# Aman-4-Real/MMTG

Measured on AMD Instinct MI355X. Metric: train tokens/sec, full MMTG config (GPT-2-base-zh decoder, 5x(img+text) 2048-d WenLan embs), higher is better.
Workload: dtype bf16; 1 GPU; Full MMTG train step: S=5 experience steps, T=15+221=236 decoder positions, GPT-2 12L/768/12H V=13317, dropout 0.1 on, MyLoss stage 3 + 0.2*KL, clip 1.0, AdamW; rows_per_gpu=64, global_rows=64, seq_len=236, parallelism=single GPU, no collective

## Files before the change

### mmtg_amd/csrc/wgrad.hip

```cpp
#include "gemm_common.h"
#include <stdlib.h>

namespace {

constexpr int WG_MAXP = 8;

struct WgProb {
    const void* A; const void* B; float* C;
    long lda, ldb, ldc;
    int M, N, tiles_m, tiles_n, tile0, m_fast;
    int bytesA, bytesB;
    int planeA, planeB;
};
struct WgArgs {
    WgProb pr[WG_MAXP];
    int n, K, kper, splits, ntiles, accumulate;
    int touch;
    float* ws;
    unsigned* cnt;
};

__device__ __forceinline__ void wg_store_band(float* C, long ldc, int M, int N, int mw0, int nw0, int h, const f32x4 (&v)[4],
                                              char* lds, int lane, bool accumulate) {
    const int g = lane >> 4, l15 = lane & 15;
// ... 283 lines not shown
    const int wr = wave >> 2, wc = wave & 3;
    int t, split, m0, n0;
    const WgProb& P = a.pr[wg_locate<256>(a, t, split, m0, n0)];
    const int M = P.M, N = P.N;
    const long lda = P.lda, ldb = P.ldb;
    const int kbeg = split * a.kper;
    const int klen = max(0, min(a.K, kbeg + a.kper) - kbeg);
    const int nk = 2 * ((klen + 127) >> 7);
    const __amdgpu_buffer_rsrc_t ra = __builtin_amdgcn_make_buffer_rsrc(const_cast<void*>(P.A), 0, P.bytesA, 0x00020000);
    const __amdgpu_buffer_rsrc_t rb = __builtin_amdgcn_make_buffer_rsrc(const_cast<void*>(P.B), 0, P.bytesB, 0x00020000);
    const int sa0 = (int)(((long)kbeg * lda + m0) * 2), sb0 = (int)(((long)kbeg * ldb + n0) * 2);
    const int stepa = (int)(64 * lda * 2), stepb = (int)(64 * ldb * 2);
    const int lA00 = wave * 1024, lA01 = (wave + 8) * 1024, lA10 = 16384 + lA00, lA11 = 16384 + lA01;
    const int lB00 = TA + lA00, lB01 = TA + lA01, lB10 = TA + lA10, lB11 = TA + lA11;
    const int vA00 = g8_voff<8>(lda, m0, M, 0, wave, lane), vA01 = g8_voff<8>(lda, m0, M, 0, wave + 8, lane);
    const int vA10 = g8_voff<8>(lda, m0, M, 1, wave, lane), vA11 = g8_voff<8>(lda, m0, M, 1, wave + 8, lane);
    const int vB00 = g8_voff<4>(ldb, n0, N, 0, wave, lane), vB01 = g8_voff<4>(ldb, n0, N, 0, wave + 8, lane);
    const int vB10 = g8_voff<4>(ldb, n0, N, 1, wave, lane), vB11 = g8_voff<4>(ldb, n0, N, 1, wave + 8, lane);
    const int kl0 = wave * 4 + (lane >> 4), kl1 = kl0 + 32;
#define G8_A0(t_) g8_issue(ra, smem + ((t_) & 1) * STAGE + lA00, smem + ((t_) & 1) * STAGE + lA01, (t_) * 64 + kl0 < klen ? vA00 : OOB, (t_) * 64 + kl1 < klen ? vA01 : OOB, sa0 + (t_) * stepa)
#define G8_A1(t_) g8_issue(ra, smem + ((t_) & 1) * STAGE + lA10, smem + ((t_) & 1) * STAGE + lA11, (t_) * 64 + kl0 < klen ? vA10 : OOB, (t_) * 64 + kl1 < klen ? vA11 : OOB, sa0 + (t_) * stepa)
#define G8_B0(t_) g8_issue(rb, smem + ((t_) & 1) * STAGE + lB00, smem + ((t_) & 1) * STAGE + lB01, (t_) * 64 + kl0 < klen ? vB00 : OOB, (t_) * 64 + kl1 < klen ? vB01 : OOB, sb0 + (t_) * stepb)
#define G8_B1(t_) g8_issue(rb, smem + ((t_) & 1) * STAGE + lB10, smem + ((t_) & 1) * STAGE + lB11, (t_) * 64 + kl0 < klen ? vB10 : OOB, (t_) * 64 + kl1 < klen ? vB11 : OOB, sb0 + (t_) * stepb)
    int oa[4], ob[2];
    ks_offsets<128, 4>(wr * 64, lane, oa);
    ks_offsets<128, 2>(wc * 32, lane, ob);
    ob[0] += TA; ob[1] += TA;

    f32x4 acc[8][4];
#pragma unroll
    for (int i = 0; i < 8; ++i)
#pragma unroll
        for (int j = 0; j < 4; ++j) acc[i][j] = f32x4{0.f, 0.f, 0.f, 0.f};

    G8_B0(0); G8_A0(0); G8_B1(0); G8_A1(0);
    G8_B0(1); G8_A0(1); G8_B1(1);
    wait_vmcnt<6>();
    asm volatile("s_barrier" ::: "memory");
    if (wr == 1) asm volatile("s_barrier" ::: "memory");

    bf16x8 fa[4][2], fb0[2][2], fb1[2][2];
#define G8_RD_A(ST, AH)                                                                                    \
    _Pragma("unroll") for (int kk = 0; kk < 2; ++kk) _Pragma("unroll") for (int i = 0; i < 4; ++i)          \
        fa[i][kk] = tr_read_pair(smem + (ST) * STAGE + (AH) * 16384, oa[i] + kk * 8192, oa[i] + kk * 8192 + 1024)
#define G8_RD_B(ST, BH, F)                                                                                 \
    _Pragma("unroll") for (int kk = 0; kk < 2; ++kk) _Pragma("unroll") for (int j = 0; j < 2; ++j)          \
        F[j][kk] = tr_read_pair(smem + (ST) * STAGE + (BH) * 16384, ob[j] + kk * 8192, ob[j] + kk * 8192 + 1024)
#define G8_TILE(ST, kt)                                                                                    \
    do {                                                                                                   \
        G8_RD_B(ST, 0, fb0);                                                                               \
        __builtin_amdgcn_sched_barrier(0);                                                                 \
        G8_RD_A(ST, 0);                                                                                    \
        G8_A1((kt) + 1);                                                                                   \
         \
        asm volatile("s_waitcnt lgkmcnt(15)" ::: "memory");                                                \
        G8_SYNC_IN(); g8_mfma<0, 0>(fa, fb0, acc); G8_SYNC_OUT();                                           \
        G8_RD_B(ST, 1, fb1);                                                                               \
        G8_B0((kt) + 2);                                                                                   \
        G8_SYNC_IN(); g8_mfma<0, 1>(fa, fb1, acc); G8_SYNC_OUT();                                           \
        G8_RD_A(ST, 1);                                                                                    \
        G8_A0((kt) + 2);                                                                                   \
        G8_SYNC_IN(); g8_mfma<1, 1>(fa, fb1, acc); G8_SYNC_OUT();                                           \
        G8_B1((kt) + 2);                                                                                   \
        wait_vmcnt<6>();                                                      \
        G8_SYNC_IN(); g8_mfma<1, 0>(fa, fb0, acc); G8_SYNC_OUT();                                           \
    } while (0)
    for (int kt = 0; kt < nk; kt += 2) {
        G8_TILE(0, kt);
        G8_TILE(1, kt + 1);
    }
#undef G8_TILE
#undef G8_RD_A
#undef G8_RD_B
#undef G8_A0
#undef G8_A1
#undef G8_B0
#undef G8_B1
    wait_vmcnt<0>();
    if (wr == 0) asm volatile("s_barrier" ::: "memory");
    asm volatile("s_barrier" ::: "memory");
    wg_reduce_store<false, 8, 256 * 256>(a, P.C, P.ldc, M, N, m0 + wr * 128, n0 + wc * 64, t, split, 8, wave, lane, acc, smem + wave * 4096);
}

}

extern "C" int mmtg_wgrad_group(int config, int n, const mmtg_wgrad_problem* probs, int K, int splits, float* ws, long ws_floats,
                                unsigned* counters, long n_counters, int accumulate, void* stream) {
    const bool x3 = (config & 2) != 0;
    const bool x3c = x3 && (config & 4) != 0;
    config &= ~6;
    MMTG_REQUIRE(config == 0 || (config == 1 && !x3),
                 "wgrad_group: config 0 (128x128 tiles), 1 (256x256 eight-phase tiles), 2 (128x128 tiles, x3 operands) or 6 (x3, combined stages)");
    const int TB = config ? 256 : 128, NWV = config ? 8 : 4, KQ = config ? 128 : 64;
    MMTG_REQUIRE(n >= 1 && n <= WG_MAXP && probs, "wgrad_group: 1..%d problems", WG_MAXP);
    MMTG_REQUIRE(K > 0 && splits >= 1, "wgrad_group: K and splits must be positive");
    WgArgs a;
    memset(&a, 0, sizeof(a));
    int tiles = 0;
    double flops = 0, bytes = 0;
    for (int i = 0; i < n; ++i) {
        const mmtg_wgrad_problem& q = probs[i];
        MMTG_REQUIRE(q.A && q.B && q.C && q.M > 0 && q.N > 0, "wgrad_group: problem %d has a null operand or an empty shape", i);
        MMTG_REQUIRE(MMTG_ALIGNED16(q.A) && MMTG_ALIGNED16(q.B) && MMTG_ALIGNED16(q.C), "wgrad_group: operands must be 16-byte aligned");
        MMTG_REQUIRE(q.lda % 8 == 0 && q.ldb % 8 == 0 && q.M % 8 == 0 && q.N % 8 == 0 && q.ldc % 4 == 0 && q.lda >= q.M && q.ldb >= q.N && q.ldc >= q.N,
                     "wgrad_group: problem %d: M, N, lda, ldb multiples of 8, ldc of 4, leading dimensions >= extents", i);
        if (x3) MMTG_REQUIRE(q.planeA % 8 == 0 && q.planeB % 8 == 0 && q.planeA >= (long)(K - 1) * q.lda + q.M && q.planeB >= (long)(K - 1) * q.ldb + q.N,
                             "wgrad_group: problem %d: an operand's lo plane must lie behind its hi plane (distance %% 8 == 0)", i);
        const long bytesA = ((x3 ? q.planeA : 0) + (long)(K - 1) * q.lda + q.M) * 2, bytesB = ((x3 ? q.planeB : 0) + (long)(K - 1) * q.ldb + q.N) * 2;
        MMTG_REQUIRE(bytesA < 0x7FFFFF00L && bytesB < 0x7FFFFF00L, "wgrad_group: operands must stay below 2 GiB");
        WgProb& p = a.pr[i];
        p.A = q.A; p.B = q.B; p.C = q.C; p.lda = q.lda; p.ldb = q.ldb; p.ldc = q.ldc; p.M = q.M; p.N = q.N;
        p.tiles_m = cdiv(q.M, TB); p.tiles_n = cdiv(q.N, TB);
        p.tile0 = tiles;
        p.m_fast = p.tiles_n > p.tiles_m;
        p.bytesA = (int)bytesA; p.bytesB = (int)bytesB;
        p.planeA = x3 ? (int)(q.planeA * 2) : 0; p.planeB = x3 ? (int)(q.planeB * 2) : 0;
        tiles += p.tiles_m * p.tiles_n;
        flops += 2.0 * q.M * q.N * (double)K;
        bytes += 2.0 * ((double)q.M * K + (double)q.N * K) + 4.0 * (double)q.M * q.N;
    }
    const int kper = cdiv(cdiv(K, splits), KQ) * KQ;
    splits = cdiv(K, kper);
    MMTG_REQUIRE(splits == 1 || (ws && counters && MMTG_ALIGNED16(ws)), "wgrad_group: split products need the workspace and the counters");
    MMTG_REQUIRE(splits == 1 || (ws_floats >= (long)tiles * splits * TB * TB && n_counters >= (long)tiles * NWV),
                 "wgrad_group: workspace needs %ld floats and %ld counters", (long)tiles * splits * TB * TB, (long)tiles * NWV);
    a.n = n; a.K = K; a.kper = kper; a.splits = splits; a.ntiles = tiles; a.accumulate = accumulate;
    a.ws = ws; a.cnt = counters;
    static const int touch = getenv("MMTG_WGRAD_TOUCH") ? atoi(getenv("MMTG_WGRAD_TOUCH")) : 0;
    a.touch = touch;
    hipStream_t s = (hipStream_t)stream;
    ProfScope prof(MMTG_PROF_GEMM_BF16, s, flops, bytes);
    static bool attr_done = false;
    static const bool fence = getenv("MMTG_WGRAD_FENCE") != nullptr;
    if (config == 1) {
        const size_t shm8 = 2 * (256 + 256) * 128;
        static bool attr8_done = false;
        if (!attr8_done) {
            if (hipFuncSetAttribute((const void*)wgrad_group_p8_kernel, hipFuncAttributeMaxDynamicSharedMemorySize, (int)shm8) != hipSuccess)
                MMTG_FAIL(MMTG_ERR_HIP, "wgrad_group: cannot raise dynamic LDS to %zu bytes", shm8);
            attr8_done = true;
        }
        hipLaunchKernelGGL(wgrad_group_p8_kernel, dim3(tiles * splits), dim3(512), shm8, s, a);
        MMTG_LAUNCH_CHECK("wgrad_group");
        return MMTG_OK;
    }
    const size_t shm = (128 + 128) * 128;
    if (!attr_done) {
        if (hipFuncSetAttribute((const void*)wgrad_group_kernel<true>, hipFuncAttributeMaxDynamicSharedMemorySize, (int)shm) != hipSuccess ||
            hipFuncSetAttribute((const void*)wgrad_group_kernel<false>, hipFuncAttributeMaxDynamicSharedMemorySize, (int)shm) != hipSuccess)
            MMTG_FAIL(MMTG_ERR_HIP, "wgrad_group: cannot raise dynamic LDS to %zu bytes", shm);
        attr_done = true;
    }
    static const int ablate = getenv("MMTG_WGRAD_ABLATE") ? atoi(getenv("MMTG_WGRAD_ABLATE")) : 0;
    if (x3c) {
        const size_t shmc = 2 * shm;
        static bool x3c_done = false;
        if (!x3c_done) {
            if (hipFuncSetAttribute((const void*)wgrad_group_kernel<false, 0, true, true>, hipFuncAttributeMaxDynamicSharedMemorySize, (int)shmc) != hipSuccess)
                MMTG_FAIL(MMTG_ERR_HIP, "wgrad_group: cannot raise dynamic LDS to %zu bytes", shmc);
            x3c_done = true;
        }
        hipLaunchKernelGGL((wgrad_group_kernel<false, 0, true, true>), dim3(tiles * splits), dim3(256), shmc, s, a);
    } else if (x3) {
        static bool x3_done = false;
        if (!x3_done) {
            if (hipFuncSetAttribute((const void*)wgrad_group_kernel<false, 0, true>, hipFuncAttributeMaxDynamicSharedMemorySize, (int)shm) != hipSuccess)
                MMTG_FAIL(MMTG_ERR_HIP, "wgrad_group: cannot raise dynamic LDS to %zu bytes", shm);
            x3_done = true;
        }
        hipLaunchKernelGGL((wgrad_group_kernel<false, 0, true>), dim3(tiles * splits), dim3(256), shm, s, a);
    } else if (ablate) {
        static bool abl_done = false;
        if (!abl_done) {
            (void)hipFuncSetAttribute((const void*)wgrad_group_kernel<false, 1>, hipFuncAttributeMaxDynamicSharedMemorySize, (int)shm);
            (void)hipFuncSetAttribute((const void*)wgrad_group_kernel<false, 2>, hipFuncAttributeMaxDynamicSharedMemorySize, (int)shm);
            abl_done = true;
        }
        if (ablate == 1) hipLaunchKernelGGL((wgrad_group_kernel<false, 1>), dim3(tiles * splits), dim3(256), shm, s, a);
        else hipLaunchKernelGGL((wgrad_group_kernel<false, 2>), dim3(tiles * splits), dim3(256), shm, s, a);
    } else if (fence) hipLaunchKernelGGL(wgrad_group_kernel<true>, dim3(tiles * splits), dim3(256), shm, s, a);
    else if (touch > 0) {
        static bool t_done = false;
        if (!t_done) { (void)hipFuncSetAttribute((const void*)wgrad_group_kernel<false, 3>, hipFuncAttributeMaxDynamicSharedMemorySize, (int)shm); t_done = true; }
        hipLaunchKernelGGL((wgrad_group_kernel<false, 3>), dim3(tiles * splits), dim3(256), shm, s, a);
    } else hipLaunchKernelGGL(wgrad_group_kernel<false>, dim3(tiles * splits), dim3(256), shm, s, a);
    MMTG_LAUNCH_CHECK("wgrad_group");
    return MMTG_OK;
}
```

### mmtg_amd/engine.py

```python
from __future__ import annotations

import contextlib
import math

import numpy as np
import torch

from . import hip
from .configs import rnn_param_shapes

ALIGN = 64


class ParamLayout:

    def __init__(self, model_cfgs, gpt2_cfg):
        S = model_cfgs["seq_len"]
        E = model_cfgs["topic"]["input_dim"]
        H = model_cfgs["topic"]["hidden_dim"]
        D = gpt2_cfg["n_embd"]
        V = gpt2_cfg["vocab_size"]
        NP = gpt2_cfg["n_positions"]
        L = gpt2_cfg["n_layer"]
        self.Vpad = (V + 127) // 128 * 128
# ... 82 lines not shown
        self.heads = model_cfgs["SELF_ATT"]["attention_heads"]
        self.P = data_cfg["topic_prompt_length"]
        self.msl = data_cfg["max_sent_length"]
        self.max_seq_length = data_cfg["max_seq_length"]
        self.two_sents = 2 * (self.msl + 2)
        self.D = gpt2_cfg["n_embd"]
        self.nH = gpt2_cfg["n_head"]
        self.L = gpt2_cfg["n_layer"]
        self.V = gpt2_cfg["vocab_size"]
        self.NP = gpt2_cfg["n_positions"]
        self.eps = gpt2_cfg.get("layer_norm_epsilon", 1e-5)
        self.pdrop = (gpt2_cfg.get("embd_pdrop", 0.1), gpt2_cfg.get("attn_pdrop", 0.1), gpt2_cfg.get("resid_pdrop", 0.1))
        self.rnn = {ch: (model_cfgs[ch]["type"], int(model_cfgs[ch]["num_layers"])) for ch in ("image", "text")}
        self.rnn_pdrop = float(model_cfgs.get("dropout", 0.0))
        for ch in ("image", "text"):
            rnn_param_shapes(model_cfgs, ch)
            if model_cfgs[ch]["input_dim"] != self.E or model_cfgs[ch]["hidden_dim"] != self.H:
                raise ValueError("The hidden dim of topic, image and text must be equal (model.py:36); this engine also takes one input dim")
        if self.D % self.nH or self.D // self.nH != 64:
            raise ValueError("the attention kernels are built for head dim 64 (n_embd=%d, n_head=%d)" % (self.D, self.nH))
        if model_cfgs["MM_ATT"]["attention_dim"] != 1:
            raise ValueError("MM_ATT.attention_dim must be 1 (the reference's broadcast at model.py:200 requires it)")


def gaussian_prior(S):
    j = np.arange(S, dtype=np.float64)
    rows = []
    for i in range(S):
        v = np.exp(-0.5 * (j - i) ** 2) / math.sqrt(2 * math.pi)
        v32 = v.astype(np.float64)
        rows.append((v32 / v32.sum()).astype(np.float32))
    return np.stack(rows)


import os as _os


def _dist_rank():
    import torch.distributed as dist
    return dist.get_rank() if dist.is_available() and dist.is_initialized() else int(_os.environ.get("RANK", "0"))


_NO_OCC4 = bool(_os.environ.get("MMTG_GEMM_NO_OCC4"))
_WG_NUM = float(_os.environ.get("MMTG_WGRAD_NUM", "760"))
_WG_CAP = int(_os.environ.get("MMTG_WGRAD_CAP", "12"))
_NO_FEW_ROWS = bool(_os.environ.get("MMTG_NO_FEW_ROWS"))
_WGRAD_SLAB = not _os.environ.get("MMTG_WGRAD_ATOMIC")
_NO_GATHER = bool(_os.environ.get("MMTG_NO_GATHER"))
_PREFETCH = int(_os.environ.get("MMTG_PREFETCH", "0"))


def _wgrad_splits(M, N, K, occ4=False, slots=512, t_iter=1.1, t_fixed=6.0):
    tiles = ((M + 127) // 128) * ((N + 127) // 128)
    if occ4 and not _NO_OCC4:
        smax = max(1, K // 256)
        s = round(_WG_NUM / tiles) if tiles < 512 else round(2520.0 / tiles)
        return int(max(1, min(smax, s, _WG_CAP)))
    best, best_t = 1, None
    for s in range(1, 33):
        if s > 1 and K // s < 256:
            break
        rounds = -(-tiles * s // slots)
        t = rounds * (K / (64.0 * s) * t_iter + t_fixed) + tiles * s * 65536 / 1.3e6
        if best_t is None or t < best_t * 0.97:
            best, best_t = s, t
    return best


_LAZY_ZERO = _os.environ.get("MMTG_FULL_ZERO_GRAD") is None
_WTE_T = _os.environ.get("MMTG_NO_WTE_T") is None
_P8T = _os.environ.get("MMTG_GEMM_P8T", "0") != "0"
_WGRAD_GROUP = _os.environ.get("MMTG_WGRAD_GROUP", "1") != "0"
_WGRAD_GROUP_SPLITS = int(_os.environ.get("MMTG_WGRAD_GROUP_SPLITS", "0"))
_GELU_GRAD = _os.environ.get("MMTG_GELU_GRAD", "0") != "0"
_DEFER_SUMS = _os.environ.get("MMTG_DEFER_SUMS", "1") != "0"
_WGRAD_TAIL = int(_os.environ.get("MMTG_WGRAD_TAIL", "8"))
_TAIL_FORK_EARLY = _os.environ.get("MMTG_WGRAD_TAIL_FORK", "loop") == "loop"
_LMHEAD_GROUP = _os.environ.get("MMTG_LMHEAD_GROUP", "1") != "0"
_LMHEAD_GROUP_SPLITS = int(_os.environ.get("MMTG_LMHEAD_GROUP_SPLITS", "0"))
_WGRAD_STREAM = _os.environ.get("MMTG_WGRAD_STREAM", "0") != "0"
_ENC_STREAMS = _os.environ.get("MMTG_ENC_STREAMS", "0") != "0"
_HYBRID_ENC_BF16 = _os.environ.get("MMTG_HYBRID_ENC_BF16", "1") != "0"
_X3_WG_CFG = 6 if _os.environ.get("MMTG_WGRAD_X3_COMBINED", "1") != "0" else 2
_WGRAD_GROUP_CFG = int(_os.environ.get("MMTG_WGRAD_GROUP_CFG", "0"))


def _group_splits(tiles, K, slots=1024):
    if _WGRAD_GROUP_SPLITS > 0:
        return _WGRAD_GROUP_SPLITS
    return int(max(1, min(slots // max(1, tiles), K // 1024, 16)))


def _group_splits_x3(tiles, K):
    if _X3_WG_CFG != 6:
        return _group_splits(tiles, K)
    if _WGRAD_GROUP_SPLITS > 0:
        return _WGRAD_GROUP_SPLITS
    s = 512 // max(1, tiles)
    if s == 0:
        s = 2048 // tiles
    return int(max(1, min(s, K // 1024, 16)))


def _wgrad_splits_p8(M, N, K, cus=256):
    if not _P8T or K % 128 or M < 256 or N < 256:
        return None
    tiles = ((M + 255) // 256) * ((N + 255) // 256)
    if tiles > cus // 2:
        return None
    units = K // 128
    s0 = max(1, min(cus // tiles, units // 4))
    per = -(-units // s0)
    return -(-units // per)


def _round_capacity(n):
    if n <= 1024:
        return 1024
    k = 1 << (int(n - 1).bit_length() - 1)
    for q in (4, 5, 6, 7, 8):
        if k * q // 4 >= n:
            return k * q // 4
    return 2 * k


def mix_seed(seed, site):
    x = (seed ^ (0x9E3779B9 * (site + 1))) & 0xFFFFFFFF
    x = ((x ^ (x >> 16)) * 0x7FEB352D) & 0xFFFFFFFF
    x = ((x ^ (x >> 15)) * 0x846CA68B) & 0xFFFFFFFF
    return (x ^ (x >> 16)) & 0xFFFFFFFF


def initial_drop_seed(rank=0):
    return mix_seed(torch.initial_seed() & 0xFFFFFFFF, 0x5EED + 7919 * rank)


class Engine:

    def __init__(self, model_cfgs, data_cfg, gpt2_cfg, master, table, dtype=hip.BF16, x3=False, hybrid=False):
        hip.lib()
        if x3 and dtype != hip.F32:
            raise ValueError("the split-precision (bf16x3) products belong to fp32 storage")
        if hybrid and not x3:
            raise ValueError("the hybrid mode (bf16x3f) is the split-precision forward with a bf16 backward: it needs x3")
        if not master.is_cuda:
            raise RuntimeError("the MMTG engine runs on an MI355X (cuda) device only -- there is no CPU path")
        self.sh = Shapes(model_cfgs, data_cfg, gpt2_cfg)
        if x3 and self.sh.D % 128:
            raise ValueError("compute_dtype='bf16x3' needs n_embd to be a multiple of 128 (got %d): use compute_dtype='f32'" % self.sh.D)
        self.layout = ParamLayout(model_cfgs, gpt2_cfg)
        assert master.numel() == self.layout.total and master.dtype == torch.float32
        self.dev = master.device
        self.dtype = dtype
        self.tdt = hip.torch_dtype(dtype)
        self.master = master
        self.grad = None
        self.wc = master if dtype == hip.F32 else torch.zeros(self.layout.total, device=self.dev, dtype=torch.bfloat16)
        self.x3 = bool(x3)
        self.hybrid = bool(hybrid)
        self.wc2 = torch.zeros(2, self.layout.total, device=self.dev, dtype=torch.bfloat16) if self.x3 else None
        self.copies_fresh = dtype == hip.F32 and not self.x3
        self._init_transposed()
        self.set_table(table)
        self.prior = torch.from_numpy(gaussian_prior(self.sh.S)).to(self.dev)
        self.ws = {}
        self._ws_tag = ""
        self.act = None
# ... 703 lines not shown
            xb = self.buf("x_cond_b", tuple(a["x"].shape), torch.bfloat16)
            hip.cast_f32_to(a["x"], xb, a["x"].numel())
        ab.update(x3=False, px3=False, gelu_grad=False, elem_mask=True, layers=layers, x_last=a["x_last_b"], hf=hi(a["hf"]), h1=h1b, x=xb, ids32=None)
        try:
            with self._as_bf16():
                self.act = ab
                seg = self._backward_decoder(ab, dlogits)
        finally:
            self.act = a
        if _HYBRID_ENC_BF16:
            ae = self._encoder_record_bf16(a)
            with self._as_bf16():
                self._backward_encoder(ae, seg, dkl)
            return
        seg32 = self.buf("d_seg32", tuple(seg.shape), torch.float32)
        hip.cast_to_f32(seg, seg32, seg.numel())
        self._backward_encoder(a, seg32, dkl)

    def _encoder_record_bf16(self, a):
        def cast(t, name):
            b = self.buf("hyb_" + name, tuple(t.shape), torch.bfloat16)
            hip.cast_f32_to(t, b, t.numel())
            return b
        ae = dict(a)
        for k in ("o", "t_ln", "t_raw", "xt"):
            ae[k] = cast(a[k], k)
        ae["alpha"] = {mod: (cast(q, "aqkv_" + mod), cast(c, "actx_" + mod), p) for mod, (q, c, p) in a["alpha"].items()}
        enc = {}
        for ch, (layers, h_ln) in a["enc"].items():
            recs = []
            for l, rec in enumerate(layers):
                r = dict(rec)
                r["h"] = cast(rec["h"], "h_%s%d" % (ch, l))
                r["inp"] = recs[l - 1]["h"] if (l > 0 and rec["inp"] is layers[l - 1]["h"]) else cast(rec["inp"], "inp_%s%d" % (ch, l))
                recs.append(r)
            enc[ch] = (recs, cast(h_ln, "hln_" + ch))
        ae["enc"] = enc
        return ae

    def backward(self, dlogits, dkl=0.0):
        a = self.act
        self.ensure_grad()
        if self._lazy is not None and not self.wgrad_overwrite:
            self.grad.zero_()
            self._lazy = None
        if self.hybrid and a.get("x3"):
            self._backward_hybrid(dlogits, dkl)
        else:
            self._backward_encoder(a, self._backward_decoder(a, dlogits), dkl)
        if self._tail_side is not None:
            torch.cuda.current_stream().wait_stream(self._tail_side)
            self._tail_side = None
        self._lazy = None

    def _backward_decoder(self, a, dlogits):
        sh = self.sh
        B, T, M, L = a["B"], a["T"], a["M"], a["L"]
        S, E, H, D, P = sh.S, sh.E, sh.H, sh.D, sh.P
        pe, pa, pr = a["pdrop"]
        Vp = self.layout.Vpad
        pre = "decoder.gpt2.transformer."
        dhf = self.buf("d_hf", (M, D))
        x3 = bool(a.get("x3"))
        if x3:
            dlp = dlogits if isinstance(dlogits, hip.Planes) else hip.split_planes(dlogits, M, Vp, self.pbuf("dlogits_p", M, Vp))
            hip.gemm_x3(dlp, hip.Planes(self.wte_t, D, Vp), dhf, M, D, Vp)
            tiles = hip.wgrad_group_sizes(((Vp, D),), 1, 0)[0]
            hs = _LMHEAD_GROUP_SPLITS or _group_splits_x3(tiles, M)
            _, nws, ncnt = hip.wgrad_group_sizes(((Vp, D),), hs, 0)
            hws = self.buf("wgrad_group_ws_head", (nws,), torch.float32) if hs > 1 else None
            hcnt = self.ws.get(("wgrad_group_cnt", torch.int32))
            if hcnt is None or hcnt.numel() < ncnt:
                hcnt = self.ws[("wgrad_group_cnt", torch.int32)] = torch.zeros(ncnt, device=self.dev, dtype=torch.int32)
            hip.wgrad_group([(dlp, a["hf"], self.Gp("wte"), Vp, D, Vp, D, D)], M, hs, hws, hcnt, accumulate=not self.wgrad_overwrite, config=_X3_WG_CFG)
            if self.wgrad_overwrite and self._ow_rec is not None:
                self._ow_rec[1].append((self.layout.pack_range["wte"][0], Vp * D))
        elif getattr(self, "wte_t", None) is not None and Vp % 128 == 0 and not self.x3:
            hip.gemm(dlogits, self.wte_t, dhf, M, D, Vp, transB=True, ldb=Vp)
        else:
            hip.gemm(dlogits, self.Wp("wte"), dhf, M, D, Vp, transB=False, ldb=D)
        if x3:
            pass
        elif _WGRAD_GROUP and _LMHEAD_GROUP and self.dtype == hip.BF16 and M >= 256 and D % 8 == 0 and Vp % 8 == 0:
            tiles = hip.wgrad_group_sizes(((Vp, D),), 1, 0)[0]
            hs = _LMHEAD_GROUP_SPLITS or _group_splits(tiles, M)
            _, nws, ncnt = hip.wgrad_group_sizes(((Vp, D),), hs, 0)
            hws = self.buf("wgrad_group_ws_head", (nws,), torch.float32) if hs > 1 else None
            hcnt = self.ws.get(("wgrad_group_cnt", torch.int32))
            if hcnt is None or hcnt.numel() < ncnt:
                hcnt = self.ws[("wgrad_group_cnt", torch.int32)] = torch.zeros(ncnt, device=self.dev, dtype=torch.int32)
            side = self._side_stream() if (_WGRAD_STREAM and pr > 0) else None
            if side is not None:
                side.wait_stream(torch.cuda.current_stream())
                with torch.cuda.stream(side):
                    hip.wgrad_group([(dlogits, a["hf"], self.Gp("wte"), Vp, D, Vp, D, D)], M, hs, hws, hcnt, accumulate=not self.wgrad_overwrite)
            else:
                hip.wgrad_group([(dlogits, a["hf"], self.Gp("wte"), Vp, D, Vp, D, D)], M, hs, hws, hcnt, accumulate=not self.wgrad_overwrite)
            if self.wgrad_overwrite and self._ow_rec is not None:
                self._ow_rec[1].append((self.layout.pack_range["wte"][0], Vp * D))
        else:
            splits = _wgrad_splits(Vp, D, M, self.dtype == hip.BF16)
            if self.dtype == hip.F32 and not self.x3 and _WGRAD_SLAB and splits > 1:
                part = self.buf("wgrad_slabs", (splits * Vp * D,), torch.float32)
                hip.gemm(dlogits, a["hf"], part, Vp, D, M, transA=True, transB=False, lda=Vp, ldb=D, ldc=D,
                         epi=hip.EPI_SPLIT, out_f32=True, splits=splits)
                hip.slab_sum(part, splits, Vp * D, self.Gp("wte"), Vp * D, accumulate=True)
            else:
                hip.gemm(dlogits, a["hf"], self.Gp("wte"), Vp, D, M, transA=True, transB=False, lda=Vp, ldb=D, ldc=D,
                         epi=hip.EPI_ATOMIC, splits=splits)
        self._defer = _DEFER_SUMS and (self.dtype == hip.BF16 or x3)
        dx = self.buf("d_resid_a", (M, D))
        dx2 = self.buf("d_resid_b", (M, D))
        group = (_WGRAD_GROUP and self.dtype == hip.BF16 and M >= 256 and D % 8 == 0) or x3
        dmask = self.buf("d_masked", (M, D)) if (pr > 0 and not x3) else None
        dmask_b = (self.buf("d_masked_b", (M, D)) if group else dmask) if (pr > 0 and not x3) else None
        if group:
            gshapes = ((D, 4 * D), (4 * D, D), (D, D), (D, 3 * D))
            gcfg = 1 if (_WGRAD_GROUP_CFG and D >= 256 and not x3) else 0
            gtiles = hip.wgrad_group_sizes(gshapes, 1, gcfg)[0]
            gsplits = _group_splits_x3(gtiles, M) if x3 else _group_splits(gtiles, M, 256 if gcfg else 1024)
            _, nws, ncnt = hip.wgrad_group_sizes(gshapes, gsplits, gcfg)
            gws = self.buf("wgrad_group_ws", (nws,), torch.float32) if gsplits > 1 else None
            gcnt = self.ws.get(("wgrad_group_cnt", torch.int32))
            if gcnt is None or gcnt.numel() < ncnt:
                gcnt = self.ws[("wgrad_group_cnt", torch.int32)] = torch.zeros(ncnt, device=self.dev, dtype=torch.int32)
        lastp = f"{pre}h.{sh.L - 1}."
        dmask_top = self.buf("d_masked_1", (M, D)) if (group and not x3 and _WGRAD_STREAM and pr > 0 and (sh.L - 1) & 1) else dmask
        ntail = min(_WGRAD_TAIL, sh.L) if (group and not _WGRAD_STREAM and (pr > 0 or x3) and self.bucket_hook is None) else 0
        tsets = {} if x3 else {t: (self.buf("d_u_t%d" % t, (M, 4 * D)), self.buf("d_masked_t%d" % t, (M, D)),
                                   self.buf("d_masked_b_t%d" % t, (M, D)), self.buf("d_qkv_t%d" % t, (M, 3 * D))) for t in range(ntail)}
        xsfx = (lambda t: "_t%d" % t if t < ntail else "") if x3 else (lambda t: "")
        if ntail == sh.L and not x3:
            dmask_top = tsets[sh.L - 1][1]
        self._tail_jobs = []
        if x3:
            dyp = self.pbuf("d_masked_p" + xsfx(sh.L - 1), M, D)
            self._ln_bwd_x3("f", dhf, a["x_last"], pre + "ln_f.weight", a["muf"], a["rsf"], None, dx, M, D, dyp,
                            drop_p=pr, drop_seed=a["layers"][sh.L - 1][13][2], colsum_key=lastp + "mlp.c_proj.bias")
        else:
            self._ln_bwd("f", dhf, a["x_last"], pre + "ln_f.weight", a["muf"], a["rsf"], None, dx, M, D,
                         dx_masked=dmask_top, drop_p=pr, drop_seed=a["layers"][sh.L - 1][13][2], colsum_key=lastp + "mlp.c_proj.bias")
        self._ready("ln_f.b")
        du = None if x3 else self.buf("d_u", (M, 4 * D))
        dm = self.buf("d_m", (M, D))
        dctx = self.buf("d_ctx", (M, D))
        dqkv = self.buf("d_qkv", (M, 3 * D))
        stream_mode = group and _WGRAD_STREAM and pr > 0 and not x3
        if stream_mode:
            side = self._side_stream()
            odd = (self.buf("d_u_1", (M, 4 * D)), self.buf("d_masked_1", (M, D)), self.buf("d_masked_b_1", (M, D)),
                   self.buf("d_qkv_1", (M, 3 * D)))
            sets = ((du, dmask, dmask_b, dqkv), odd)
            wdone = {}
        da = self.buf("d_a", (M, D))
        delta = self.buf("attn_delta", (M, sh.nH), torch.float32)
        dq32 = self.buf("attn_dq32", (hip.attn_bwd_x3_dq_floats(B, T, D),) if x3 else (M, D), torch.float32)
        for l in range(sh.L - 1, -1, -1):
            p = f"{pre}h.{l}."
            (xin, mu1, rs1, a1, qkv, ctx, lse, xmid, mu2, rs2, m2, u, gact, s, ctxp) = a["layers"][l]
            if stream_mode:
                du, dmask, dmask_b, dqkv = sets[l & 1]
            if l in tsets:
                du, dmask, dmask_b, dqkv = tsets[l]
            if x3:
                bands = self.buf("d_u_bands_%d" % l if self._defer else "d_u_bands", ((M + 63) // 64, 4 * D), torch.float32)
                dup = self.pbuf("d_u_p" + xsfx(l), M, 4 * D)
                self._dgrad_x3(dyp, p + "mlp.c_proj.weight", None, M, planes=dup, ldc=4 * D, epi=hip.EPI_DGELU, aux=u, ldaux=4 * D, aux2=bands)
                if self._defer and bands.shape[0] <= 2048:
                    self._defer_sum(bands, 4 * D, bands.shape[0], 4 * D, self.G(p + "mlp.c_fc.bias"))
                else:
                    hip.colsum(bands, bands.shape[0], 4 * D, self.G(p + "mlp.c_fc.bias"))
                self._dgrad_x3(dup, p + "mlp.c_fc.weight", dm, M)
                dy2p = self.pbuf("d_masked_b_p" + xsfx(l), M, D)
                self._ln_bwd_x3("%d_2" % l, dm, xmid, p + "ln_2.weight", mu2, rs2, dx, dx2, M, D, dy2p,
                                drop_p=pr, drop_seed=s[1], colsum_key=p + "attn.c_proj.bias")
                dqkvp = self.pbuf("d_qkv_p" + xsfx(l), M, 3 * D)
                dctxp = self.pbuf("d_ctx_p", M, D)
                self._dgrad_x3(dy2p, p + "attn.c_proj.weight", None, M, planes=dctxp, ldc=D, epi=hip.EPI_ROWDOT, aux=ctx, ldaux=D, aux2=delta)
                nkv, nq = B * (-(-T // 128)), -(-M // 16)
                brows = self._defer and nkv <= 2048 and nq <= 2048
                bws = self.buf("attn_dbias_x3_%d" % l if brows else "attn_dbias_x3", (hip.attn_bwd_x3_ws(B, T, D),), torch.float32)
                hip.attn_bwd_x3(qkv, a["keep"], ctx, dctxp, lse, delta, dq32, dqkvp, B, T, sh.nH, D // sh.nH, drop_p=pa, drop_seed=s[0],
                                dbias=None if brows else self.G(p + "attn.c_attn.bias"), delta_ready=True, dbias_ws=bws)
                if brows:
                    self._defer_sum(bws, 3 * D, nkv, 2 * D, self.G(p + "attn.c_attn.bias")[D:], offset=D)
                    self._defer_sum(bws, D, nq, D, self.G(p + "attn.c_attn.bias"), offset=nkv * 3 * D)
                self._dgrad_x3(dqkvp, p + "attn.c_attn.weight", da, M)
                keys = (p + "mlp.c_fc.weight", p + "mlp.c_proj.weight", p + "attn.c_proj.weight", p + "attn.c_attn.weight")
                probs = [(m2, dup, self.G(keys[0]), D, 4 * D), (gact, dyp, self.G(keys[1]), 4 * D, D),
                         (ctxp, dy2p, self.G(keys[2]), D, D), (a1, dqkvp, self.G(keys[3]), D, 3 * D)]
                if l < ntail:
                    self._tail_jobs.append((probs, M, gsplits, gws, gcnt, not self.wgrad_overwrite, _X3_WG_CFG))
                else:
                    hip.wgrad_group(probs, M, gsplits, gws, gcnt, accumulate=not self.wgrad_overwrite, config=_X3_WG_CFG)
                if self.wgrad_overwrite and self._ow_rec is not None:
                    self._ow_rec[1].extend((self.layout.entries[k][0], self.layout.entries[k][2]) for k in keys)
                if l > 0:
                    dyp = self.pbuf("d_masked_p" + xsfx(l - 1), M, D)
                    self._ln_bwd_x3("%d_1" % l, da, xin, p + "ln_1.weight", mu1, rs1, dx2, dx, M, D, dyp,
                                    drop_p=pr, drop_seed=a["layers"][l - 1][13][2], colsum_key=f"{pre}h.{l - 1}.mlp.c_proj.bias")
                else:
# ... 270 lines not shown
```

### mmtg_amd/hip.py

```python
from __future__ import annotations

import ctypes as C
import os

import torch

from .constraints import check_mirostat, check_warp

F32, BF16 = 0, 1
ABI_VERSION = 12
EPI_NONE, EPI_GELU, EPI_TANH, EPI_RESID, EPI_DGELU, EPI_DTANH, EPI_ATOMIC, EPI_ROWDOT = range(8)
GEMM_NO_TR, GEMM_REGSTAGE, GEMM_SKINNY, GEMM_NO_SKINNY, GEMM_WIDE, GEMM_NO_WIDE = 1, 2, 4, 8, 16, 32
GEMM_PERSIST, GEMM_NO_PERSIST, GEMM_ROW_ORDER, GEMM_OCC4, GEMM_NO_OCC4, GEMM_COL_BLOCK, GEMM_P256, GEMM_NO_P8, GEMM_P8 = 64, 128, 256, 512, 1024, 2048, 4096, 8192, 16384
GEMM_GELU_GRAD = 32768
GEMM_P8_288 = 65536
GEMM_AUX2_BF16 = 131072
PROF_CATS = ["gemm_bf16", "gemm_f32", "attn_fwd", "attn_bwd", "layernorm", "embed", "loss",
             "optim", "encoder", "decode", "misc"]

_LIB_PATH = os.path.join(os.path.dirname(os.path.abspath(__file__)), "libmmtg_hip.so")
_lib = None

_vp, _i, _l, _f, _u = C.c_void_p, C.c_int, C.c_long, C.c_float, C.c_uint

# ... 576 lines not shown
    _check(lib().mmtg_rnn_cell_bwd(dt(da), kind, _p(rows), ld_rows, _p(part), _p(save), _p(c_prev), _p(h), ld_h, _p(dc), int(dc_in),
                                   _p(da), ld_da, B, H, _stream()), "rnn_cell_bwd")


def alpha_attn_fwd(qkv, prior, ctx, probs, kl, B, S, H, heads):
    _check(lib().mmtg_alpha_attn_fwd(dt(qkv), _p(qkv), _p(prior), _p(ctx), _p(probs), _p(kl), B, S, H, heads,
                                     _stream()), "alpha_attn_fwd")


def alpha_attn_bwd(qkv, prior, probs, dctx, dkl, dqkv, B, S, H, heads):
    _check(lib().mmtg_alpha_attn_bwd(dt(qkv), _p(qkv), _p(prior), _p(probs), _p(dctx), float(dkl), _p(dqkv),
                                     B, S, H, heads, _stream()), "alpha_attn_bwd")


def beta_fuse_fwd(topic, img, txt, att_w, att_b, o, a, B, S, H):
    _check(lib().mmtg_beta_fuse_fwd(dt(topic), _p(topic), _p(img), _p(txt), _p(att_w), _p(att_b), _p(o), _p(a),
                                    B, S, H, _stream()), "beta_fuse_fwd")


_beta_ws = {}


def beta_fuse_bwd(topic, img, txt, att_w, a, d_o, dtopic, dimg, dtxt, datt_w, datt_b, B, S, H):
    need = int(lib().mmtg_beta_fuse_bwd_ws(B, S, H))
    key = (d_o.device, need, _stream())
    ws = _beta_ws.get(key)
    if ws is None:
        if len(_beta_ws) > 64:
            _beta_ws.clear()
        ws = _beta_ws[key] = torch.empty(need, device=d_o.device, dtype=torch.float32)
    _check(lib().mmtg_beta_fuse_bwd(dt(topic), _p(topic), _p(img), _p(txt), _p(att_w), _p(a), _p(d_o), _p(dtopic),
                                    _p(dimg), _p(dtxt), _p(datt_w), _p(datt_b), B, S, H, _p(ws), ws.numel(), _stream()), "beta_fuse_bwd")


def prefetch(t, sink, workgroups=256, stream=None):
    _check(lib().mmtg_prefetch(_p(t), t.numel() * t.element_size(), int(workgroups), _p(sink),
                               _stream() if stream is None else stream.cuda_stream), "prefetch")


_sumsq_ws = {}


def sumsq(x, n, out):
    need = int(lib().mmtg_sumsq_ws(n))
    key = (x.device, need, _stream())
    ws = _sumsq_ws.get(key)
    if ws is None:
        ws = _sumsq_ws[key] = torch.empty(need, device=x.device, dtype=torch.float32)
    _check(lib().mmtg_sumsq(_p(x), n, _p(out), _p(ws), need, _stream()), "sumsq")


def adamw(p, g, m, v, p_bf16, n, lr, beta1, beta2, eps, wd, step, normsq, max_norm, grad_scale=1.0, count=None, p_lo=None):
    _check(lib().mmtg_adamw(_p(p), _p(g), _p(m), _p(v), _p(p_bf16), _p(p_lo), n, float(lr), float(beta1), float(beta2),
                            float(eps), float(wd), int(step), _p(normsq), float(max_norm), float(grad_scale),
                            _p(count), _stream()), "adamw")


def cast_f32_to(src, dst, n):
    _check(lib().mmtg_cast_f32_to(dt(dst), _p(src), _p(dst), n, _stream()), "cast_f32_to")


def cast_pad_rows(src, lds, dst, ldd, rows, cols):
    _check(lib().mmtg_cast_pad_rows(dt(dst), _p(src), lds, _p(dst), ldd, rows, cols, _stream()), "cast_pad_rows")


def cast_to_f32(src, dst, n):
    _check(lib().mmtg_cast_to_f32(dt(src), _p(src), _p(dst), n, _stream()), "cast_to_f32")


def axpy_f32(y, x, a, n):
    _check(lib().mmtg_axpy_f32(_p(y), _p(x), float(a), n, _stream()), "axpy_f32")


def slab_sum(part, splits, stride, dst, n, accumulate=True):
    _check(lib().mmtg_slab_sum(_p(part), splits, stride, _p(dst), int(accumulate), n, _stream()), "slab_sum")


class WgradProblem(C.Structure):
    _fields_ = [("A", C.c_void_p), ("lda", C.c_long), ("B", C.c_void_p), ("ldb", C.c_long),
                ("C", C.c_void_p), ("ldc", C.c_long), ("M", C.c_int), ("N", C.c_int),
                ("planeA", C.c_long), ("planeB", C.c_long)]


def wgrad_group_sizes(shapes, splits, config=0):
    tb, nw = (256, 8) if config else (128, 4)
    tiles = sum(((M + tb - 1) // tb) * ((N + tb - 1) // tb) for (M, N) in shapes)
    return tiles, tiles * splits * tb * tb, tiles * nw


def wgrad_group(problems, K, splits, ws, counters, accumulate=False, config=0):
    arr = (WgradProblem * len(problems))()
    for i, pr in enumerate(problems):
        A, B, C_, M, N = pr[:5]
        lda, ldb, ldc = (pr[5:8] if len(pr) >= 8 else (M, N, N))
        if config & 2:
            arr[i] = WgradProblem(_p(A.t), lda, _p(B.t), ldb, _p(C_), ldc, M, N, A.plane, B.plane)
        else:
            arr[i] = WgradProblem(_p(A), lda, _p(B), ldb, _p(C_), ldc, M, N, 0, 0)
    _check(lib().mmtg_wgrad_group(int(config), len(problems), C.addressof(arr), int(K), int(splits), _p(ws), 0 if ws is None else ws.numel(),
                                  _p(counters), 0 if counters is None else counters.numel(), int(accumulate), _stream()), "wgrad_group")


def transpose_batch(src, dst, desc, n, max_rows, max_cols):
    _check(lib().mmtg_transpose_batch(dt(src), _p(src), _p(dst), _p(desc), n, max_rows, max_cols, _stream()), "transpose_batch")


def logits_process_argmax(logits, ldl, V, generated, ldg, gen_len, temperature, rep_penalty, nxt, B):
    _check(lib().mmtg_logits_process_argmax(_p(logits), ldl, V, _p(generated), ldg, _p(gen_len),
                                            float(temperature), float(rep_penalty), _p(nxt), B, _stream()),
           "logits_process_argmax")


def logits_process_sample(logits, ldl, V, generated, ldg, gen_len, temperature, rep_penalty, top_k, top_p, uniforms, nxt, B,
                          filtered=None):
    _check(lib().mmtg_logits_process_sample(_p(logits), ldl, V, _p(generated), ldg, _p(gen_len), float(temperature),
                                            float(rep_penalty), int(top_k), float(top_p), _p(uniforms), _p(nxt), _p(filtered),
                                            B, _stream()), "logits_process_sample")


def logits_process_sample_warp(logits, ldl, V, generated, ldg, gen_len, temperature, rep_penalty, top_k, top_p, uniforms, nxt, B,
                               min_p=0.0, typical_p=1.0, epsilon_cutoff=0.0, eta_cutoff=0.0, filtered=None):
    warp = check_warp(min_p, typical_p, epsilon_cutoff, eta_cutoff)
    _check(lib().mmtg_logits_process_sample_warp(_p(logits), ldl, V, _p(generated), ldg, _p(gen_len), float(temperature),
                                                 float(rep_penalty), int(top_k), float(top_p), *warp, _p(uniforms), _p(nxt),
                                                 _p(filtered), B, _stream()), "logits_process_sample_warp")


def logits_process_sample_mirostat(logits, ldl, V, generated, ldg, gen_len, temperature, rep_penalty, top_k, top_p, uniforms, nxt, B,
                                   mirostat_tau, mirostat_eta, mu, surprise=None, min_p=0.0, typical_p=1.0, epsilon_cutoff=0.0,
                                   eta_cutoff=0.0, filtered=None):
    warp = check_warp(min_p, typical_p, epsilon_cutoff, eta_cutoff)
    tau, eta = check_mirostat(mirostat_tau, mirostat_eta)
    if tau == 0.0:
        raise ValueError("mirostat_tau must be in (0, 32] here: 0 (off) is logits_process_sample_warp")
    _check(lib().mmtg_logits_process_sample_mirostat(_p(logits), ldl, V, _p(generated), ldg, _p(gen_len), float(temperature),
                                                     float(rep_penalty), int(top_k), float(top_p), *warp, _p(uniforms), _p(nxt),
                                                     _p(filtered), B, tau, eta, _p(mu), _p(surprise), _stream()),
           "logits_process_sample_mirostat")


def decode_embed(table, seq, c, x, pos, tpw_type, tpw_mask, type_out, keep, B, P, S, E, two_sents, V, sent, max_sent_num):
    _check(lib().mmtg_decode_embed(dt(table), _p(table), _p(seq), seq.stride(0), _p(c), _p(x), _p(pos), _p(tpw_type),
                                   _p(tpw_mask), _p(type_out), _p(keep), keep.stride(0), B, P, S, E, two_sents, V, sent,
                                   max_sent_num, _stream()), "decode_embed")


def decode_embed_add(g, wpe, wte, type_ids, pos, h, B, D, stats=None):
    _check(lib().mmtg_decode_embed_add(dt(g), _p(g), _p(wpe), _p(wte), _p(type_ids), _p(pos), _p(h), B, D, _p(stats), _stream()),
           "decode_embed_add")


DG_NP = 32


def decode_gemm(mode, A, W, C_, M, N, K, bias=None, colsum=None, stats_in=None, np_in=0, eps=1e-5, act=EPI_NONE, out_f32=False,
                resid=None, stats_out=None, splits=1, ws=None, counters=None, lda=None, ldw=None, ldc=None, ldr=None,
                emb_pos=None, emb_type=None, type_ids=None, pos=None):
    _check(lib().mmtg_decode_gemm(int(mode), M, N, K, _p(A), K if lda is None else lda, _p(W), K if ldw is None else ldw, _p(C_),
                                  N if ldc is None else ldc, _p(bias), _p(colsum), _p(stats_in), int(np_in), float(eps), int(act),
                                  int(out_f32), _p(resid), N if ldr is None else ldr, _p(stats_out), int(splits), _p(ws),
                                  0 if ws is None else ws.numel(), _p(counters), 0 if counters is None else counters.numel(),
                                  _p(emb_pos), _p(emb_type), _p(type_ids), _p(pos), _stream()), "decode_gemm")


def decode_gemm_x3(mode, A, W, M, N, K, C_=None, Cp=None, ldc=None, bias=None, colsum=None, stats_in=None, np_in=0, eps=1e-5, act=EPI_NONE,
                   resid=None, ldr=None, stats_out=None, splits=1, ws=None, counters=None, emb_pos=None, emb_type=None, type_ids=None, pos=None):
    _check(lib().mmtg_decode_gemm_x3(int(mode), M, N, K, _p(A.t), A.ld, A.plane, _p(W.t), W.ld, W.plane, _p(C_), N if ldc is None else ldc,
                                     0 if Cp is None else _p(Cp.t), 0 if Cp is None else Cp.ld, 0 if Cp is None else Cp.plane,
# ... 442 lines not shown
```

Measured before the change: 1.034 million tokens/s.

## Add 16-wave triple-buffered ring kernel for grouped weight-gradient GEMMs and enable by default

Adds a new 256x256-tile wgrad kernel with 1024 threads that streams K-slices of A and B into a three-stage LDS ring via direct buffer-to-LDS loads, reading operands with transposing LDS reads and one barrier per stage. It becomes the default for the per-layer grouped wgrad and also for the LM-head wte gradient, replacing the 128x128 four-wave kernel, with fewer split slots. The aim is better data reuse and overlap of global loads with MFMA work. In exchange it runs one block per CU with large LDS use and fewer tiles, which may reduce parallelism for small shapes.

```diff
diff --git a/mmtg_amd/csrc/wgrad.hip b/mmtg_amd/csrc/wgrad.hip
--- a/mmtg_amd/csrc/wgrad.hip
+++ b/mmtg_amd/csrc/wgrad.hip
@@ -389,6 +389,100 @@
     wg_reduce_store<false, 8, 256 * 256>(a, P.C, P.ldc, M, N, m0 + wr * 128, n0 + wc * 64, t, split, 8, wave, lane, acc, smem + wave * 4096);
 }
 
+__device__ __forceinline__ void wg_raw_barrier() { asm volatile("s_waitcnt lgkmcnt(0)\n\ts_barrier" ::: "memory"); }
+
+__device__ __forceinline__ void wgr_read_stage(unsigned base, const int (&oa)[4], const int (&ob)[4], bf16x8 (&fa)[4], bf16x8 (&fb)[4]) {
+    s16x4 al[4], ah[4], bl[4], bh[4];
+    unsigned pa[4], pb[4];
+#pragma unroll
+    for (int i = 0; i < 4; ++i) { pa[i] = base + (unsigned)oa[i]; pb[i] = base + (unsigned)ob[i]; }
+    asm volatile(
+        "ds_read_b64_tr_b16 %0, %16\n\t"
+        "ds_read_b64_tr_b16 %1, %16 offset:2048\n\t"
+        "ds_read_b64_tr_b16 %2, %17\n\t"
+        "ds_read_b64_tr_b16 %3, %17 offset:2048\n\t"
+        "ds_read_b64_tr_b16 %4, %18\n\t"
+        "ds_read_b64_tr_b16 %5, %18 offset:2048\n\t"
+        "ds_read_b64_tr_b16 %6, %19\n\t"
+        "ds_read_b64_tr_b16 %7, %19 offset:2048\n\t"
+        "ds_read_b64_tr_b16 %8, %20 offset:16384\n\t"
+        "ds_read_b64_tr_b16 %9, %20 offset:18432\n\t"
+        "ds_read_b64_tr_b16 %10, %21 offset:16384\n\t"
+        "ds_read_b64_tr_b16 %11, %21 offset:18432\n\t"
+        "ds_read_b64_tr_b16 %12, %22 offset:16384\n\t"
+        "ds_read_b64_tr_b16 %13, %22 offset:18432\n\t"
+        "ds_read_b64_tr_b16 %14, %23 offset:16384\n\t"
+        "ds_read_b64_tr_b16 %15, %23 offset:18432\n\t"
+        "s_waitcnt lgkmcnt(0)"
+        : "=&v"(al[0]), "=&v"(ah[0]), "=&v"(al[1]), "=&v"(ah[1]), "=&v"(al[2]), "=&v"(ah[2]), "=&v"(al[3]), "=&v"(ah[3]),
+          "=&v"(bl[0]), "=&v"(bh[0]), "=&v"(bl[1]), "=&v"(bh[1]), "=&v"(bl[2]), "=&v"(bh[2]), "=&v"(bl[3]), "=&v"(bh[3])
+        : "v"(pa[0]), "v"(pa[1]), "v"(pa[2]), "v"(pa[3]), "v"(pb[0]), "v"(pb[1]), "v"(pb[2]), "v"(pb[3])
+        : "memory");
+#pragma unroll
+    for (int i = 0; i < 4; ++i) {
+        fa[i] = __builtin_shufflevector(__builtin_bit_cast(bf16x4, al[i]), __builtin_bit_cast(bf16x4, ah[i]), 0, 1, 2, 3, 4, 5, 6, 7);
+        fb[i] = __builtin_shufflevector(__builtin_bit_cast(bf16x4, bl[i]), __builtin_bit_cast(bf16x4, bh[i]), 0, 1, 2, 3, 4, 5, 6, 7);
+    }
+}
+
+__global__ __launch_bounds__(1024, 1) void wgrad_group_ring_kernel(WgArgs a) {
+    constexpr int TB = 256, BK = 32, IMG = BK * TB * 2, STAGE = 2 * IMG;
+    extern __shared__ __attribute__((aligned(16))) char smem[];
+    const int tid = threadIdx.x, lane = tid & 63;
+    const int wave = __builtin_amdgcn_readfirstlane(tid >> 6);
+    const int wm = wave >> 2, wn = wave & 3;
+    int t, split, m0, n0;
+    const WgProb& P = a.pr[wg_locate<TB>(a, t, split, m0, n0)];
+    const int M = P.M, N = P.N;
+    const long lda = P.lda, ldb = P.ldb;
+    const int kbeg = split * a.kper;
+    const int klen = max(0, min(a.K, kbeg + a.kper) - kbeg);
+    const int ns = (klen + BK - 1) / BK;
+    const __amdgpu_buffer_rsrc_t ra = __builtin_amdgcn_make_buffer_rsrc(const_cast<void*>(P.A), 0, P.bytesA, 0x00020000);
+    const __amdgpu_buffer_rsrc_t rb = __builtin_amdgcn_make_buffer_rsrc(const_cast<void*>(P.B), 0, P.bytesB, 0x00020000);
+    const int sa0 = (int)(((long)kbeg * lda + m0) * 2), sb0 = (int)(((long)kbeg * ldb + n0) * 2);
+    const int stepa = (int)((long)BK * lda * 2), stepb = (int)((long)BK * ldb * 2);
+    const int va = dma_voff<true, TB>(lda, m0, M, BK, wave, lane);
+    const int vb = dma_voff<true, TB>(ldb, n0, N, BK, wave, lane);
+    const int kl = wave * 2 + (lane >> 5);
+    int oa[4], ob[4];
+    ks_offsets<TB, 4>(wm * 64, lane, oa);
+    ks_offsets<TB, 4>(wn * 64, lane, ob);
+    f32x4 acc[4][4];
+#pragma unroll
+    for (int i = 0; i < 4; ++i)
+#pragma unroll
+        for (int j = 0; j < 4; ++j) acc[i][j] = f32x4{0.f, 0.f, 0.f, 0.f};
+
+    auto issue = [&](int st, int slot) {
+        const bool in = st < ns, ok = st * BK + kl < klen;
+        const int soa = __builtin_amdgcn_readfirstlane(in ? sa0 + st * stepa : 0);
+        const int sob = __builtin_amdgcn_readfirstlane(in ? sb0 + st * stepb : 0);
+        __builtin_amdgcn_raw_ptr_buffer_load_lds(ra, LDS_PTR(void, smem + slot + wave * 1024), 16, ok ? va : OOB, soa, 0, 0);
+        __builtin_amdgcn_raw_ptr_buffer_load_lds(rb, LDS_PTR(void, smem + slot + IMG + wave * 1024), 16, ok ? vb : OOB, sob, 0, 0);
+    };
+    issue(0, 0);
+    issue(1, STAGE);
+    const unsigned lds0 = (unsigned)(unsigned long)LDS_PTR(char, smem);
+    int rd = 0, wr = 2 * STAGE;
+    for (int s = 0; s < ns; ++s) {
+        wait_vmcnt<2>();
+        wg_raw_barrier();
+        issue(s + 2, wr);
+        bf16x8 fa[4], fb[4];
+        wgr_read_stage(lds0 + rd, oa, ob, fa, fb);
+#pragma unroll
+        for (int i = 0; i < 4; ++i)
+#pragma unroll
+            for (int j = 0; j < 4; ++j) mma16(fb[j], fa[i], acc[i][j]);
+        wr = rd;
+        rd = rd == 2 * STAGE ? 0 : rd + STAGE;
+    }
+    wait_vmcnt<0>();
+    wg_raw_barrier();
+    wg_reduce_store<false, 4, TB * TB>(a, P.C, P.ldc, M, N, m0 + wm * 64, n0 + wn * 64, t, split, 16, wave, lane, acc, smem + wave * 4096);
+}
+
 }
 
 extern "C" int mmtg_wgrad_group(int config, int n, const mmtg_wgrad_problem* probs, int K, int splits, float* ws, long ws_floats,
@@ -396,9 +490,9 @@
     const bool x3 = (config & 2) != 0;
     const bool x3c = x3 && (config & 4) != 0;
     config &= ~6;
-    MMTG_REQUIRE(config == 0 || (config == 1 && !x3),
-                 "wgrad_group: config 0 (128x128 tiles), 1 (256x256 eight-phase tiles), 2 (128x128 tiles, x3 operands) or 6 (x3, combined stages)");
-    const int TB = config ? 256 : 128, NWV = config ? 8 : 4, KQ = config ? 128 : 64;
+    MMTG_REQUIRE(config == 0 || ((config == 1 || config == 8) && !x3),
+                 "wgrad_group: config 0 (128x128 tiles), 1 (256x256 eight-phase tiles), 8 (256x256 tiles, 16-wave ring), 2 (128x128 tiles, x3 operands) or 6 (x3, combined stages)");
+    const int TB = config ? 256 : 128, NWV = config == 8 ? 16 : config ? 8 : 4, KQ = config == 1 ? 128 : 64;
     MMTG_REQUIRE(n >= 1 && n <= WG_MAXP && probs, "wgrad_group: 1..%d problems", WG_MAXP);
     MMTG_REQUIRE(K > 0 && splits >= 1, "wgrad_group: K and splits must be positive");
     WgArgs a;
@@ -451,6 +545,18 @@
         MMTG_LAUNCH_CHECK("wgrad_group");
         return MMTG_OK;
     }
+    if (config == 8) {
+        const size_t shmr = 3 * 2 * 32 * 256 * 2;
+        static bool attrr_done = false;
+        if (!attrr_done) {
+            if (hipFuncSetAttribute((const void*)wgrad_group_ring_kernel, hipFuncAttributeMaxDynamicSharedMemorySize, (int)shmr) != hipSuccess)
+                MMTG_FAIL(MMTG_ERR_HIP, "wgrad_group: cannot raise dynamic LDS to %zu bytes", shmr);
+            attrr_done = true;
+        }
+        hipLaunchKernelGGL(wgrad_group_ring_kernel, dim3(tiles * splits), dim3(1024), shmr, s, a);
+        MMTG_LAUNCH_CHECK("wgrad_group");
+        return MMTG_OK;
+    }
     const size_t shm = (128 + 128) * 128;
     if (!attr_done) {
         if (hipFuncSetAttribute((const void*)wgrad_group_kernel<true>, hipFuncAttributeMaxDynamicSharedMemorySize, (int)shm) != hipSuccess ||
diff --git a/mmtg_amd/engine.py b/mmtg_amd/engine.py
--- a/mmtg_amd/engine.py
+++ b/mmtg_amd/engine.py
@@ -188,7 +188,13 @@
 _ENC_STREAMS = _os.environ.get("MMTG_ENC_STREAMS", "0") != "0"
 _HYBRID_ENC_BF16 = _os.environ.get("MMTG_HYBRID_ENC_BF16", "1") != "0"
 _X3_WG_CFG = 6 if _os.environ.get("MMTG_WGRAD_X3_COMBINED", "1") != "0" else 2
-_WGRAD_GROUP_CFG = int(_os.environ.get("MMTG_WGRAD_GROUP_CFG", "0"))
+_WGRAD_GROUP_CFG = int(_os.environ.get("MMTG_WGRAD_GROUP_CFG", "2"))
+
+
+def _group_cfg(D, x3=False):
+    if x3 or D < 256 or _WGRAD_GROUP_CFG not in (1, 2):
+        return 0
+    return hip.WGRAD_RING if _WGRAD_GROUP_CFG == 2 else 1
 
 
 def _group_splits(tiles, K, slots=1024):
@@ -1058,9 +1064,10 @@
         if x3:
             pass
         elif _WGRAD_GROUP and _LMHEAD_GROUP and self.dtype == hip.BF16 and M >= 256 and D % 8 == 0 and Vp % 8 == 0:
-            tiles = hip.wgrad_group_sizes(((Vp, D),), 1, 0)[0]
-            hs = _LMHEAD_GROUP_SPLITS or _group_splits(tiles, M)
-            _, nws, ncnt = hip.wgrad_group_sizes(((Vp, D),), hs, 0)
+            hcfg = hip.WGRAD_RING if _group_cfg(D) == hip.WGRAD_RING else 0
+            tiles = hip.wgrad_group_sizes(((Vp, D),), 1, hcfg)[0]
+            hs = _LMHEAD_GROUP_SPLITS or _group_splits(tiles, M, 256 if hcfg else 1024)
+            _, nws, ncnt = hip.wgrad_group_sizes(((Vp, D),), hs, hcfg)
             hws = self.buf("wgrad_group_ws_head", (nws,), torch.float32) if hs > 1 else None
             hcnt = self.ws.get(("wgrad_group_cnt", torch.int32))
             if hcnt is None or hcnt.numel() < ncnt:
@@ -1069,9 +1076,9 @@
             if side is not None:
                 side.wait_stream(torch.cuda.current_stream())
                 with torch.cuda.stream(side):
-                    hip.wgrad_group([(dlogits, a["hf"], self.Gp("wte"), Vp, D, Vp, D, D)], M, hs, hws, hcnt, accumulate=not self.wgrad_overwrite)
+                    hip.wgrad_group([(dlogits, a["hf"], self.Gp("wte"), Vp, D, Vp, D, D)], M, hs, hws, hcnt, accumulate=not self.wgrad_overwrite, config=hcfg)
             else:
-                hip.wgrad_group([(dlogits, a["hf"], self.Gp("wte"), Vp, D, Vp, D, D)], M, hs, hws, hcnt, accumulate=not self.wgrad_overwrite)
+                hip.wgrad_group([(dlogits, a["hf"], self.Gp("wte"), Vp, D, Vp, D, D)], M, hs, hws, hcnt, accumulate=not self.wgrad_overwrite, config=hcfg)
             if self.wgrad_overwrite and self._ow_rec is not None:
                 self._ow_rec[1].append((self.layout.pack_range["wte"][0], Vp * D))
         else:
@@ -1092,7 +1099,7 @@
         dmask_b = (self.buf("d_masked_b", (M, D)) if group else dmask) if (pr > 0 and not x3) else None
         if group:
             gshapes = ((D, 4 * D), (4 * D, D), (D, D), (D, 3 * D))
-            gcfg = 1 if (_WGRAD_GROUP_CFG and D >= 256 and not x3) else 0
+            gcfg = _group_cfg(D, x3)
             gtiles = hip.wgrad_group_sizes(gshapes, 1, gcfg)[0]
             gsplits = _group_splits_x3(gtiles, M) if x3 else _group_splits(gtiles, M, 256 if gcfg else 1024)
             _, nws, ncnt = hip.wgrad_group_sizes(gshapes, gsplits, gcfg)
diff --git a/mmtg_amd/hip.py b/mmtg_amd/hip.py
--- a/mmtg_amd/hip.py
+++ b/mmtg_amd/hip.py
@@ -682,8 +682,11 @@
                 ("planeA", C.c_long), ("planeB", C.c_long)]
 
 
+WGRAD_RING = 8
+
+
 def wgrad_group_sizes(shapes, splits, config=0):
-    tb, nw = (256, 8) if config else (128, 4)
+    tb, nw = (256, 16) if config == WGRAD_RING else (256, 8) if config else (128, 4)
     tiles = sum(((M + tb - 1) // tb) * ((N + tb - 1) // tb) for (M, N) in shapes)
     return tiles, tiles * splits * tb * tb, tiles * nw
 
```

After: 1.083 million tokens/s, median of 6. +4.7%, better.
